# mengshanfeng/stencil-2

Measured on AMD Instinct MI355X. Metric: Jacobi3D Gcells/s (512^3/GPU weak scaling; halo-exchange GB/s in extra), higher is better.
Workload: dtype fp32

## Files before the change

csrc/include/stencil/kernels/stencil_ops.hpp:

```cpp
#pragma once
#include <cstdint>
#include <vector>

#include "stencil/core/geometry.hpp"
#include "stencil/domain/local_domain.hpp"

namespace stencil {

enum class StencilKind : int {
  Jacobi = 0,
  Astaroth = 1,
};

struct Spheres {
  bool enabled = false;
  Dim3 hot, cold;
  int64_t radius = 0;
  static Spheres jacobi(const Rect3 &cReg) {
    Spheres s;
    s.enabled = true;
    s.hot = Dim3(cReg.lo.x + (cReg.hi.x - cReg.lo.x) / 3, (cReg.lo.y + cReg.hi.y) / 2, (cReg.lo.z + cReg.hi.z) / 2);
    s.cold = Dim3(cReg.lo.x + (cReg.hi.x - cReg.lo.x) * 2 / 3, (cReg.lo.y + cReg.hi.y) / 2, (cReg.lo.z + cReg.hi.z) / 2);
    s.radius = (cReg.hi.x - cReg.lo.x) / 10;
    return s;
  }
};

struct StencilTune {
  int variant = 2;
  static constexpr int kMfma = 8;
  int ty = 2;
  int zchunk = 0;
  int nw = 8;
  int x3sched = 1;
  int x3parts = 0;
  float x3sphw = 0.45f;
  float x2sphw = 0.15f;
  bool x3sphchunk = true;
  int x3left = 3;
  bool x2early = true;
  int x2row = 1;
  int x2sched = 1;
  int x2xfast = 0;
  int x2reserve = 8;
  int reserveCUs = 0;
  bool x2lockstep = true;
  bool zslabRow = true;
  bool xcdRemap = true;
  bool nontemporal = true;
  bool alternateZ = true;
  int wrap = 0;
  uint64_t *publish = nullptr;
  uint64_t *blockClock = nullptr;
  int publishDepth = 0;
};
bool stencil7x2_row_kernel_used(const LocalDomain &dom, int64_t qi, const Rect3 &region, const StencilTune &tune);
int stencil7x2_wrappable_axes(const LocalDomain &dom, int64_t qi, int x2row = 1);

struct ForwardTarget {
  Dim3 dir;
  const LocalDomain *dst;
  Dim3 offset;
};

class HaloForwarder {
public:
  HaloForwarder(const LocalDomain &src, int64_t qi, const std::vector<ForwardTarget> &targets);
  ~HaloForwarder();
  HaloForwarder(const HaloForwarder &) = delete;
  HaloForwarder &operator=(const HaloForwarder &) = delete;
  const int *wm() const { return wm_; }
  const int *wp() const { return wp_; }
  int num_targets() const { return n_; }
  uint32_t mask(int parity) const { return mask_[parity]; }
  int64_t delta(int parity, int k) const { return delta_[parity][k]; }
  bool has_rest() const { return hasRest_; }
  void forward_rest(int parity, hipStream_t stream) const;
  static bool supported(const LocalDomain &dom, int64_t qi);

private:
  int wm_[3] = {0, 0, 0}, wp_[3] = {0, 0, 0};
  int n_ = 0;
  int dev_ = -1;
  uint32_t mask_[2] = {0, 0};
  int64_t delta_[2][27] = {};
  CopyPlan rest_[2];
  bool hasRest_ = false;
};
// ... 11 lines not shown
                    hipStream_t stream, const StencilTune &tune = StencilTune(), const HaloForwarder *fwd = nullptr);
bool stencil7x2_supported(const LocalDomain &dom, int64_t qi);
void stencil7x2_apply(const LocalDomain &dom, int64_t qi, const Rect3 &region, StencilKind kind, const Spheres &sph,
                      hipStream_t stream, const StencilTune &tune = StencilTune());
bool stencil7x3_supported(const LocalDomain &dom, int64_t qi, const Rect3 &region, const StencilTune &tune);
bool stencil7x3_apply(const LocalDomain &dom, int64_t qi, const Rect3 &region, StencilKind kind, const Spheres &sph,
                      hipStream_t stream, const StencilTune &tune);
void stencil7x2_apply_regions(const LocalDomain &dom, int64_t qi, const std::vector<Rect3> &regions, StencilKind kind,
                              const Spheres &sph, hipStream_t stream, int wrap = 0);
void stencil7x2_apply_exterior(const LocalDomain &dom, int64_t qi, const Rect3 &interior, StencilKind kind,
                               const Spheres &sph, hipStream_t stream, const StencilTune &tune = StencilTune());
struct X2Schedule {
  int parts = 0;
  int64_t blocks = 0;
  int rounds = 1;
};
inline X2Schedule x2_lockstep_schedule(int64_t slots, int64_t cols, int64_t nz, bool rounds = true) {
  X2Schedule r;
  if (slots < 4 || cols < 1) return r;
  if (cols > slots && rounds) {
    if (nz < 16) return r;
    r.rounds = int((cols + slots - 1) / slots);
    r.parts = 1;
    r.blocks = (cols + r.rounds - 1) / r.rounds;
    return r;
  }
  const int64_t P = (slots / 4 > cols || slots % cols == 0) ? slots / cols : 4;
  const int64_t cm = cols < slots / P ? cols : slots / P;
  if (cm < 1 || nz < 64 || nz / P < 16) return r;
  r.parts = int(P);
  r.blocks = P * cm;
  if (rounds && P == 4 && cm < cols && cols % 2 == 0) {
    const int64_t ch = cols / 2, P2 = slots / ch;
    if (P2 >= 2 && nz / P2 >= 16 && 16 * P2 * ch >= 15 * slots) {
      r.parts = int(P2);
      r.blocks = P2 * ch;
      r.rounds = 2;
    }
  }
  return r;
}

struct X3Schedule {
  int seg = 1, parts = 0;
  int64_t blocks = 0;
  int rounds = 1;
};
X3Schedule stencil7x3_schedule(bool xh, int64_t cols, int64_t nz, int64_t slots, const StencilTune &tune,
                               bool publishing);
struct X3LaunchInfo {
  bool supported = false;
  bool xh = false, ragged = false;
  int64_t cols = 0, slots = 0;
  int seg = 0, parts = 0;
  int64_t blocks = 0;
  int rounds = 0;
};
X3LaunchInfo stencil7x3_launch_info(const LocalDomain &dom, int64_t qi, const Rect3 &region, StencilKind kind,
                                    const Spheres &sph, const StencilTune &tune);

int stencil7_wrappable_axes(const LocalDomain &dom, int64_t qi);
bool stencil7_mfma_supported(const LocalDomain &dom, int64_t qi);
void stencil7_mfma_apply(const LocalDomain &dom, int64_t qi, const Rect3 &region, StencilKind kind, const Spheres &sph,
                         hipStream_t stream, const StencilTune &tune = StencilTune());
void stencil7_apply_regions(const LocalDomain &dom, int64_t qi, const std::vector<Rect3> &regions, StencilKind kind,
                            const Spheres &sph, hipStream_t stream, const StencilTune &tune = StencilTune());

void jacobi_init(const LocalDomain &dom, int64_t qi, const Rect3 &region, hipStream_t stream);
void astaroth_init(const LocalDomain &dom, int64_t qi, double period, hipStream_t stream);
void fill_value(const LocalDomain &dom, int64_t qi, double value, bool curr, hipStream_t stream);

}
```

csrc/python/bindings.cpp:

```cpp
#include <pybind11/functional.h>
#include <pybind11/pybind11.h>
#include <pybind11/stl.h>

#include <cstring>

#include "stencil/comm/proc_group.hpp"
#include "stencil/comm/ipc_event.hpp"
#include "stencil/comm/rccl_comm.hpp"
#include "stencil/domain/distributed_domain.hpp"
#include "stencil/kernels/copy.hpp"
#include "stencil/kernels/stencil_ops.hpp"
#include "stencil/models/stencil_model.hpp"
#include "stencil/rt/build_info.hpp"
#include "stencil/rt/statistics.hpp"
#include "stencil/topo/gpu_topology.hpp"
#include "stencil/topo/partition.hpp"
#include "stencil/topo/placement.hpp"
#include "stencil/topo/qap.hpp"

namespace py = pybind11;
using namespace stencil;

extern "C" {
struct DLDevice {
// ... 677 lines not shown
        py::arg("dd"), py::arg("domain"), py::arg("qi"));
  m.def("stencil7x2_apply",
        [](DistributedDomain &dd, size_t di, int64_t q, const Rect3 &region, StencilKind kind, bool spheres,
           uintptr_t stream, const StencilTune &tune) {
          STENCIL_REQUIRE(stencil7x2_supported(dd.domains().at(di), q),
                          "fused pairs need a device fp32/fp64 quantity, face radii >= 2 and the aligned layout");
          const Spheres s = spheres ? Spheres::jacobi(dd.get_compute_region()) : Spheres();
          stencil7x2_apply(dd.domains().at(di), q, region, kind, s, reinterpret_cast<hipStream_t>(stream), tune);
        },
        py::arg("dd"), py::arg("domain"), py::arg("qi"), py::arg("region"), py::arg("kind"), py::arg("spheres"),
        py::arg("stream"), py::arg("tune"), py::call_guard<py::gil_scoped_release>());
  py::class_<X3PlanInfo>(m, "X3PlanInfo")
      .def_readonly("parts", &X3PlanInfo::parts)
      .def_readonly("blocks", &X3PlanInfo::blocks)
      .def_readonly("groups", &X3PlanInfo::groups)
      .def_readonly("lockstep_groups", &X3PlanInfo::lockstepGroups)
      .def_readonly("rounds", &X3PlanInfo::rounds)
      .def_readonly("tabled", &X3PlanInfo::tabled)
      .def_readonly("steps", &X3PlanInfo::steps)
      .def_readonly("zb", &X3PlanInfo::zb)
      .def_readonly("l0", &X3PlanInfo::l0)
      .def_readonly("l1", &X3PlanInfo::l1)
      .def_readonly("odd", &X3PlanInfo::odd);
  m.def(
      "stencil7x3_plan",
      [](py::handle size, bool jacobi, py::object tune, int slots) {
        return stencil7x3_plan(to_dim3(size), jacobi, tune.is_none() ? StencilTune() : tune.cast<StencilTune>(), slots);
      },
      py::arg("size"), py::arg("jacobi"), py::arg("tune") = py::none(), py::arg("slots") = 256);
  m.def(
      "stencil7x3_schedule",
      [](bool xh, int64_t cols, int64_t nz, int64_t slots, py::object tune, bool publishing) {
        const X3Schedule r = stencil7x3_schedule(xh, cols, nz, slots,
                                                 tune.is_none() ? StencilTune() : tune.cast<StencilTune>(), publishing);
        return py::make_tuple(r.seg, r.parts, r.blocks, r.rounds);
      },
      py::arg("xh"), py::arg("cols"), py::arg("nz"), py::arg("slots"), py::arg("tune") = py::none(),
      py::arg("publishing") = false,
      "launch schedule of a fused-triple sweep (no GPU): (seg, parts, blocks, rounds) for the XH form (xh, columns with "
      "x halos) or the whole-row form over cols (row group, column) pairs of nz planes on `slots` resident blocks; seg "
      "1 = balanced split, 2 = lockstep parts plus second segments, 3 = lockstep rounds (XH form, not publishing)");
  m.def(
      "stencil7x3_launch_info",
      [](DistributedDomain &dd, size_t di, int64_t q, StencilKind kind, bool spheres, const StencilTune &tune) {
        const Spheres s = spheres ? Spheres::jacobi(dd.get_compute_region()) : Spheres();
        const LocalDomain &d = dd.domains().at(di);
        const X3LaunchInfo r = stencil7x3_launch_info(d, q, d.get_compute_region(), kind, s, tune);
        py::dict o;
        o["supported"] = r.supported;
        o["form"] = !r.supported ? "none" : (r.xh ? "xh" : "wrap");
        o["ragged"] = r.ragged;
        o["cols"] = r.cols;
        o["slots"] = r.slots;
        o["seg"] = r.seg;
        o["parts"] = r.parts;
        o["blocks"] = r.blocks;
        o["rounds"] = r.rounds;
        return o;
      },
      py::arg("dd"), py::arg("domain"), py::arg("qi"), py::arg("kind"), py::arg("spheres"), py::arg("tune"));
  m.def(
      "x2_lockstep_schedule",
      [](int64_t slots, int64_t cols, int64_t nz) {
        const X2Schedule r = x2_lockstep_schedule(slots, cols, nz);
        return py::make_tuple(r.parts, r.blocks, r.rounds);
      },
      py::arg("slots"), py::arg("cols"), py::arg("nz"),
      "lockstep schedule of the whole-row / two-chunk-column fused pairs: (z parts per row group, blocks, rounds of "
      "whole columns); (0, 0, 1) = balanced split");
  m.def("jacobi_spheres", [](const Rect3 &cReg) {
    Spheres s = Spheres::jacobi(cReg);
    return py::make_tuple(s.hot, s.cold, s.radius);
  });

  py::class_<StencilTune>(m, "StencilTune")
      .def(py::init<>())
      .def_readwrite("variant", &StencilTune::variant)
      .def_readwrite("ty", &StencilTune::ty)
      .def_readwrite("zchunk", &StencilTune::zchunk)
      .def_readwrite("xcd_remap", &StencilTune::xcdRemap)
      .def_readwrite("nontemporal", &StencilTune::nontemporal)
      .def_readwrite("alternate_z", &StencilTune::alternateZ)
      .def_readwrite("nw", &StencilTune::nw)
      .def_readwrite("x3sched", &StencilTune::x3sched)
      .def_readwrite("x2early", &StencilTune::x2early)
      .def_readwrite("x3parts", &StencilTune::x3parts)
      .def_readwrite("x3sphw", &StencilTune::x3sphw)
      .def_readwrite("x3sphchunk", &StencilTune::x3sphchunk)
      .def_readwrite("x3left", &StencilTune::x3left)
      .def_readwrite("x2sphw", &StencilTune::x2sphw)
      .def_property(
          "block_clock", [](const StencilTune &t) { return reinterpret_cast<uintptr_t>(t.blockClock); },
          [](StencilTune &t, uintptr_t p) { t.blockClock = reinterpret_cast<uint64_t *>(p); })
      .def_readwrite("x2row", &StencilTune::x2row)
      .def_readwrite("x2sched", &StencilTune::x2sched)
      .def_readwrite("x2reserve", &StencilTune::x2reserve)
      .def_readwrite("wrap", &StencilTune::wrap)
      .def_readwrite("x2lockstep", &StencilTune::x2lockstep)
      .def_readwrite("zslab_row", &StencilTune::zslabRow)
      .def_readwrite("x2xfast", &StencilTune::x2xfast);
  py::class_<StencilModelConfig>(m, "StencilModelConfig")
      .def(py::init<>())
      .def_readwrite("size", &StencilModelConfig::size)
      .def_readwrite("kind", &StencilModelConfig::kind)
      .def_readwrite("radius", &StencilModelConfig::radius)
      .def_readwrite("all_directions", &StencilModelConfig::allDirections)
      .def_readwrite("quantities", &StencilModelConfig::quantities)
      .def_readwrite("fp64", &StencilModelConfig::fp64)
      .def_readwrite("methods", &StencilModelConfig::methods)
      .def_readwrite("placement", &StencilModelConfig::placement)
      .def_readwrite("axis_cost", &StencilModelConfig::axisCost)
      .def_readwrite("partition", &StencilModelConfig::partition)
      .def_readwrite("gpus", &StencilModelConfig::gpus)
      .def_readwrite("overlap", &StencilModelConfig::overlap)
      .def_readwrite("auto_overlap", &StencilModelConfig::autoOverlap)
      .def_readwrite("use_graph", &StencilModelConfig::useGraph)
      .def_readwrite("forward", &StencilModelConfig::forward)
      .def_readwrite("temporal", &StencilModelConfig::temporal)
      .def_readwrite("wrap_self", &StencilModelConfig::wrapSelf)
      .def_readwrite("x_halo_align", &StencilModelConfig::xHaloAlign)
      .def_readwrite("shared_halo_line", &StencilModelConfig::sharedHaloLine)
      .def_readwrite("interior_align", &StencilModelConfig::interiorAlign)
      .def_readwrite("row_pad_lines", &StencilModelConfig::rowPadLines)
      .def_readwrite("wrap_axes_mask", &StencilModelConfig::wrapAxesMask)
      .def_readwrite("local_interior", &StencilModelConfig::localInterior)
      .def_readwrite("overlap_mode", &StencilModelConfig::overlapMode)
      .def_readwrite("transport", &StencilModelConfig::transport)
      .def_readwrite("self_test", &StencilModelConfig::selfTest)
      .def_property(
          "backend", [](const StencilModelConfig &c) { return c.backend; },
          [](StencilModelConfig &c, Backend b) {
            c.backend = b;
            c.setBackend = true;
          })
      .def_readwrite("tune", &StencilModelConfig::tune)
      .def_readwrite("astaroth_period", &StencilModelConfig::astarothPeriod);
  py::class_<StencilModel, std::shared_ptr<StencilModel>>(m, "StencilModel")
      .def(py::init([](const StencilModelConfig &c, std::shared_ptr<comm::ProcGroup> pg) {
             py::gil_scoped_release r;
// ... 36 lines not shown
```

csrc/src/kernels/stencil7x3.hip:

```cpp
#include <hip/hip_runtime.h>

#include <algorithm>
#include <map>
#include <mutex>
#include <utility>
#include <vector>
#include <cmath>
#include <cstring>

#include "stencil/kernels/stencil_ops.hpp"
#include "stencil/rt/hip_check.hpp"
#include "stencil_common.hpp"
#include "stencil_wave.hpp"

namespace stencil {

struct X3Seg {
  uint32_t s, e, s2, e2;
  bool odd;
  bool odd2;
};
template <typename T>
__device__ __forceinline__ X3Seg x3_segments(const StencilArgs<T> &a, const ZPartBounds &B, uint32_t lb, uint32_t nb,
                                             uint32_t ncols, uint32_t gy, uint32_t nzt) {
// ... 407 lines not shown
            for (int h = 0; h < H; ++h) {
              U1b[h] = U1c[h];
              U1c[h] = U1a[h];
              U2b[h] = U2c[h];
              U2c[h] = U2a[h];
            }
            if constexpr (EDGE) {
              U1Eb = U1Ec;
              U1Ec = U1Ea;
            }
            ++t;
            return true;
          };
          using I0 = std::integral_constant<int, 0>;
          using I1 = std::integral_constant<int, 1>;
          using I2 = std::integral_constant<int, 2>;
          using I3 = std::integral_constant<int, 3>;
          using L1 = std::integral_constant<int, (RM < 1 ? RM : 1)>;
          using L2 = std::integral_constant<int, (RM < 2 ? RM : 2)>;
          using LR = std::integral_constant<int, RM>;
          step(I0{}, L1{});
          step(I1{}, L1{});
          step(I2{}, L2{});
          step(I3{}, L2{});
          while (step(I0{}, LR{}) && step(I1{}, LR{}) && step(I2{}, LR{}) && step(I3{}, LR{})) {
          }
        };
        if (down)
          march(std::true_type{});
        else
          march(std::false_type{});
      }
    }
  };
  const unsigned long long clk0 = a.clk ? wall_clock64() : 0;
  const int role = (w >= 3 && w < NW - 3) ? 3 : ((w >= 2 && w < NW - 2) ? 2 : ((w >= 1 && w < NW - 1) ? 1 : 0));
  if (role == 3)
    body(std::integral_constant<int, 3>{});
  else if (role == 2)
    body(std::integral_constant<int, 2>{});
  else if (role == 1)
    body(std::integral_constant<int, 1>{});
  else
    body(std::integral_constant<int, 4>{});
  if (a.clk) {
    __syncthreads();
    if (lane == 0 && w == 0) {
      a.clk[2 * lb] = clk0;
      a.clk[2 * lb + 1] = wall_clock64();
    }
  }
}

template <int KIND, bool PUB>
__global__ __launch_bounds__(64 * 12, 3) __attribute__((amdgpu_waves_per_eu(3, 3))) void
stencil7x3_wrap_kernel(StencilArgs<float> a, ZPartBounds zbounds) {
  constexpr int NW = 12;
  using T = float;
  using NV = nf4;
  constexpr int V = 4, H = 2;
  constexpr int CS = 64 * V;
  constexpr int LS = V;
  constexpr int YO = NW - 6;
  constexpr int NC = 4;
  __shared__ NV cs[2][NW][H][64];
  __shared__ NV us[2][NW][H][64];
  __shared__ NV vs[2][NW][H][64];

  const uint32_t nb = gridDim.x;
  const uint32_t lb = a.remap ? xcd_remap(blockIdx.x, nb) : blockIdx.x;
  const int lane = threadIdx.x;
  const int w = __builtin_amdgcn_readfirstlane(int(threadIdx.y));
  const uint32_t nzt = uint32_t(a.hiz - a.loz);
  const X3Seg sg = x3_segments(a, zbounds, lb, nb, uint32_t(a.gy), uint32_t(a.gy), nzt);
  const bool lane0 = lane == 0, lane63 = lane == 63;
  const int wA = w > 0 ? w - 1 : 0, wB = w < NW - 1 ? w + 1 : NW - 1;
  const int xb = a.lox + lane * LS;
  const int zwn = a.wn[2], zwlo = a.wlo[2], zwhi = a.wlo[2] + a.wn[2];
  const __amdgpu_buffer_rsrc_t srcRsrc =
      __builtin_amdgcn_make_buffer_rsrc(const_cast<float *>(a.src), 0, -1, 0x00020000);
  auto zcl = [&](int zz) {
    zz += zz < zwlo ? zwn : 0;
    zz -= zz >= zwhi ? zwn : 0;
    return zz < 0 ? 0 : (zz > a.rawZm1 ? a.rawZm1 : zz);
  };
  auto body = [&](auto roleTag) {
    constexpr int R = decltype(roleTag)::value;
    bool odd = sg.odd;
    const bool pubOrder = PUB;
    for (int pp = 0; pp < 2; ++pp) {
      const int pass = pubOrder ? 1 - pp : pp;
      uint32_t s = pass == 0 ? sg.s : sg.s2;
      const uint32_t e = pass == 0 ? sg.e : sg.e2;
      if (pass == 1 && !pubOrder) odd = sg.odd2;
      while (s < e) {
        const uint32_t by = s / nzt;
        const int zo = int(s - by * nzt);
        const int nzs = int(min(nzt - uint32_t(zo), e - s));
        s += uint32_t(nzs);
        const int zs = a.loz + zo;
        const int ze = zs + nzs;
        bool down = pass == 0 && sg.odd;
        if (!pubOrder) {
          down = odd != (a.flip != 0);
          odd = !odd;
        }
        const int yblk = a.loy + YO * int(by);
        const int y = yblk - 3 + w;
        if (yblk >= a.hiy) continue;
        const bool outRow = R == 3 && y < a.hiy;
        int yw = y < a.wlo[1] ? y + a.wn[1] : (y >= a.wlo[1] + a.wn[1] ? y - a.wn[1] : y);
        yw = yw < 0 ? 0 : (yw > a.rawYm1 ? a.rawYm1 : yw);
        const uint32_t rowoff = uint32_t((yw * int64_t(a.px) + xb) * int64_t(sizeof(T)));
        const uint32_t outoff = uint32_t((y * int64_t(a.px) + xb) * int64_t(sizeof(T)));

        const int yh = a.r1sq - (y - a.hy) * (y - a.hy), yc = a.r1sq - (y - a.cy) * (y - a.cy);
        struct RowSph {
          int Dh, Dc;
          bool hit;
        };
        auto row_sph = [&](int P) -> RowSph {
          RowSph r{0, 0, false};
          if (KIND == 0) {
            r.Dh = yh - (P - a.hz) * (P - a.hz);
            r.Dc = yc - (P - a.cz) * (P - a.cz);
            r.hit = max(r.Dh, r.Dc) > 0;
          }
          return r;
        };
        auto sphere_row = [&](const RowSph &rs, NV(&o)[H]) {
          if (KIND == 0 && rs.hit) {
            const int Dh = rs.Dh, Dc = rs.Dc;
#pragma unroll
            for (int h = 0; h < H; ++h)
#pragma unroll
              for (int k = 0; k < V; ++k) {
                const int x = xb + h * CS + k;
                const bool hot = (x - a.hx) * (x - a.hx) < Dh;
                const bool cold = (x - a.cx) * (x - a.cx) < Dc;
                o[h][k] = hot ? T(1) : (cold ? T(0) : o[h][k]);
              }
          }
        };
        auto row_update = [&](const NV(&cm)[H], const NV(&up)[H], const NV(&dn)[H], const NV(&zp)[H], const NV(&zm)[H],
                              NV(&o)[H]) -> T {
          static_assert(H == 2, "two chunks per lane");
          const T r30 = rot_prev(cm[0][V - 1]), r31 = rot_prev(cm[1][V - 1]);
          const T l00 = rot_next(cm[0][0]), l01 = rot_next(cm[1][0]);
#pragma unroll
          for (int h = 0; h < H; ++h) {
            const T left = h == 0 ? (lane0 ? r31 : r30) : (lane0 ? r30 : r31);
            const T right = h == 0 ? (lane63 ? l01 : l00) : (lane63 ? l00 : l01);
            NV vpx, vmx;
#pragma unroll
            for (int k = 0; k < V; ++k) {
              vpx[k] = k < V - 1 ? cm[h][k + 1] : right;
              vmx[k] = k > 0 ? cm[h][k - 1] : left;
            }
            o[h] = div6v<T, NV, V>(sum6v<T, KIND>(vpx, vmx, dn[h], up[h], zp[h], zm[h]));
          }
          return T(1);
        };

        auto march = [&](auto downTag) {
          constexpr bool DOWN = decltype(downTag)::value;
          constexpr int dz = DOWN ? -1 : 1;
          const int z0 = DOWN ? ze - 1 : zs;
          NV C[NC][H];
          NV U1a[H], U1b[H], U1c[H];
          NV U2a[H], U2b[H], U2c[H];
          auto load_row = [&](int zz, int k) {
            const uint32_t po = uint32_t(zcl(zz)) * uint32_t(a.pxy) * uint32_t(sizeof(T));
#pragma unroll
            for (int h = 0; h < H; ++h)
              C[k][h] = __builtin_bit_cast(
                  NV, __builtin_amdgcn_raw_buffer_load_b128(srcRsrc, rowoff + uint32_t(h * CS * int(sizeof(T))), po, 0));
          };
          {
            const int zw = z0 - 3 * dz;
#pragma unroll
            for (int k = 0; k < NC - 1; ++k) load_row(zw + k * dz, k);
#pragma unroll
            for (int h = 0; h < H; ++h) {
              cs[0][w][h][lane] = C[1][h];
              U1a[h] = U1b[h] = U1c[h] = U2a[h] = U2b[h] = U2c[h] = C[1][h];
            }
            __syncthreads();
          }
          int buf = 0;
          int t = -4;
          auto step = [&](auto phase, auto lvTag) -> bool {
            constexpr int k = decltype(phase)::value;
            constexpr int LV = decltype(lvTag)::value;
            constexpr int s0 = k % NC, s1 = (k + 1) % NC, s2 = (k + 2) % NC, sn = (k + NC - 1) % NC;
            if (t >= nzs) return false;
            const int z = z0 + t * dz;
            load_row(z + NC * dz, sn);
            NV o[H];
            auto levels = [&]() {
              NV A1[H], B1[H], A2[H], B2[H], A3[H], B3[H];
              auto rd = [&](NV(&sh)[2][NW][H][64], NV(&A)[H], NV(&B)[H]) {
#pragma unroll
                for (int h = 0; h < H; ++h) {
                  A[h] = sh[buf][wA][h][lane];
                  B[h] = sh[buf][wB][h][lane];
                }
              };
              if constexpr (LV >= 1) {
                rd(cs, A1, B1);
                (void)row_update(C[s1], A1, B1, DOWN ? C[s0] : C[s2], DOWN ? C[s2] : C[s0], U1a);
                sphere_row(row_sph(z + 2 * dz), U1a);
#pragma unroll
                for (int h = 0; h < H; ++h) cs[buf ^ 1][w][h][lane] = C[s2][h];
#pragma unroll
                for (int h = 0; h < H; ++h) us[buf ^ 1][w][h][lane] = U1a[h];
              }
              if constexpr (LV >= 2) {
                rd(us, A2, B2);
                (void)row_update(U1c, A2, B2, DOWN ? U1b : U1a, DOWN ? U1a : U1b, U2a);
                sphere_row(row_sph(z + dz), U2a);
#pragma unroll
                for (int h = 0; h < H; ++h) vs[buf ^ 1][w][h][lane] = U2a[h];
              }
              if constexpr (LV >= 3) {
                rd(vs, A3, B3);
                (void)row_update(U2c, A3, B3, DOWN ? U2b : U2a, DOWN ? U2a : U2b, o);
                sphere_row(row_sph(z), o);
              }
            };
            levels();
            if constexpr (LV >= 3) {
              char *dp = outRow ? reinterpret_cast<char *>(a.dst + int64_t(z) * a.pxy) + outoff
                                : a.sink + lane * LS * int(sizeof(T));
#pragma unroll
              for (int h = 0; h < H; ++h) {
                NV *q = reinterpret_cast<NV *>(dp + h * CS * int(sizeof(T)));
                if (a.nt)
                  __builtin_nontemporal_store(o[h], q);
                else
                  *q = o[h];
              }
            }
            const int nbuf = buf ^ 1;
            if constexpr (LV < 1)
#pragma unroll
              for (int h = 0; h < H; ++h) cs[nbuf][w][h][lane] = C[s2][h];
            const bool pubStep = PUB && t >= 0 && (z < a.pubLo || z >= a.pubHi);
            if (pubStep) asm volatile("s_waitcnt vmcnt(0)" ::: "memory");
            __syncthreads();
            if (pubStep && lane == 0 && w == 0) {
              __builtin_amdgcn_fence(__ATOMIC_RELEASE, "");
              const unsigned long long cells =
                  (unsigned long long)(min(YO, a.hiy - yblk)) * (unsigned long long)(a.hix - a.lox);
              __hip_atomic_fetch_add(a.pub, cells, __ATOMIC_RELAXED, __HIP_MEMORY_SCOPE_SYSTEM);
            }
            buf = nbuf;
#pragma unroll
            for (int h = 0; h < H; ++h) {
              U1b[h] = U1c[h];
              U1c[h] = U1a[h];
              U2b[h] = U2c[h];
              U2c[h] = U2a[h];
            }
            ++t;
            return true;
          };
          using I0 = std::integral_constant<int, 0>;
          using I1 = std::integral_constant<int, 1>;
          using I2 = std::integral_constant<int, 2>;
          using I3 = std::integral_constant<int, 3>;
          using L1 = std::integral_constant<int, (R < 1 ? R : 1)>;
          using L2 = std::integral_constant<int, (R < 2 ? R : 2)>;
          using LR = std::integral_constant<int, R>;
          step(I0{}, L1{});
          step(I1{}, L1{});
          step(I2{}, L2{});
          step(I3{}, L2{});
          while (step(I0{}, LR{}) && step(I1{}, LR{}) && step(I2{}, LR{}) && step(I3{}, LR{})) {
          }
        };
        if (down)
          march(std::true_type{});
        else
          march(std::false_type{});
      }
    }
  };
  const unsigned long long clk0 = a.clk ? wall_clock64() : 0;
  const int role = (w >= 3 && w < NW - 3) ? 3 : ((w >= 2 && w < NW - 2) ? 2 : ((w >= 1 && w < NW - 1) ? 1 : 0));
  if (role == 3)
    body(std::integral_constant<int, 3>{});
  else if (role == 2)
    body(std::integral_constant<int, 2>{});
  else if (role == 1)
    body(std::integral_constant<int, 1>{});
  else
    body(std::integral_constant<int, 0>{});
  if (a.clk) {
    __syncthreads();
    if (lane == 0 && w == 0) {
      a.clk[2 * lb] = clk0;
      a.clk[2 * lb + 1] = wall_clock64();
    }
  }
}

template <typename T, int KIND> static const void *x3_wrap_kernel_ptr() {
  if constexpr (std::is_same<T, float>::value)
    return (const void *)stencil7x3_wrap_kernel<KIND, false>;
  else
    return nullptr;
}
template <typename T, int KIND> using X3XhKernel = void (*)(StencilArgs<T>, ZPartBounds);
template <typename T, int KIND, bool BIG, bool PUB> static X3XhKernel<T, KIND> x3_xh_kernel_ptr(bool rag) {
  return rag ? stencil7x3_xh_kernel<T, KIND, BIG, PUB, true> : stencil7x3_xh_kernel<T, KIND, BIG, PUB, false>;
}
template <typename T, int KIND> static X3XhKernel<T, KIND> x3_xh_kernel_ptr(bool big, bool pub, bool rag) {
  return big ? (pub ? x3_xh_kernel_ptr<T, KIND, true, true>(rag) : x3_xh_kernel_ptr<T, KIND, true, false>(rag))
             : (pub ? x3_xh_kernel_ptr<T, KIND, false, true>(rag) : x3_xh_kernel_ptr<T, KIND, false, false>(rag));
}

static int64_t x3_resident_blocks(const void *kernel, int threads) {
  static std::map<const void *, int64_t> cache;
  static std::mutex mu;
  std::lock_guard<std::mutex> lk(mu);
  auto it = cache.find(kernel);
  if (it != cache.end()) return it->second;
  int dev = 0, perCU = 0, cus = 256;
  (void)hipGetDevice(&dev);
  if (hipDeviceGetAttribute(&cus, hipDeviceAttributeMultiprocessorCount, dev) != hipSuccess) cus = 256;
  if (hipOccupancyMaxActiveBlocksPerMultiprocessor(&perCU, kernel, threads, 0) != hipSuccess || perCU <= 0) perCU = 1;
  (void)hipGetLastError();
  const int64_t r = int64_t(perCU) * cus;
  cache[kernel] = r;
  return r;
}

static std::map<int, char *> gX3Sinks;
static std::mutex gX3SinkMu;
static char *x3_sink(int dev, bool create) {
  std::lock_guard<std::mutex> lk(gX3SinkMu);
  char *&p = gX3Sinks[dev];
  if (!p && create) {
    int cur = 0;
    HIP_CHECK(hipGetDevice(&cur));
    HIP_CHECK(hipSetDevice(dev));
    HIP_CHECK(hipMalloc(reinterpret_cast<void **>(&p), 4096));
    HIP_CHECK(hipSetDevice(cur));
  }
  return p;
}

static int64_t x3_column_cells(int64_t elemSize) { return 2 * 64 * (16 / elemSize); }

bool stencil7x3_supported(const LocalDomain &dom, int64_t qi, const Rect3 &region, const StencilTune &tune) {
  if (dom.backend() != Backend::Device) return false;
  const int64_t es = dom.elem_size(qi);
  const bool f32 = dom.dtype(qi) == DType::F32 || (dom.dtype(qi) == DType::Bytes && es == 4);
  const bool f64 = dom.dtype(qi) == DType::F64 || (dom.dtype(qi) == DType::Bytes && es == 8);
  if (!f32 && !f64) return false;
  const Radius &rad = dom.radius();
  const Dim3 n = dom.size();
  const int wrapm = tune.wrap & 7;
  if (wrapm & 1) {
// ... 28 lines not shown
  X2Schedule ls = x2_lockstep_schedule(slots, cols, nz, rounds);
  if (tune.x3sched == 1) {
    ls = X2Schedule();
    double best = 1e30;
    for (int64_t P = 2; P <= 8; ++P) {
      if (tune.x3parts > 0 && P != tune.x3parts) continue;
      const int64_t cm = std::min<int64_t>(cols, slots / P);
      if (cm < 1 || nz / P < 16) continue;
      const int64_t blocksP = P * cm, left = cols - cm;
      const double cost = double(nz) / double(P) + 4 + (left > 0 ? double(left * nz) / double(blocksP) + 4 : 0);
      if (cost < best - 1e-9) {
        best = cost;
        ls.parts = int(P);
        ls.blocks = blocksP;
      }
    }
  }
  if (tune.x3sched == 1 && cols > slots && rounds) {
    ls = X2Schedule();
    double best = 1e30;
    for (int64_t R = (cols + slots - 1) / slots; R <= 4 * ((cols + slots - 1) / slots); ++R)
      for (int64_t P = 1; P <= 4; ++P) {
        const int64_t cm = (cols + R - 1) / R;
        if (P * cm > slots || nz / P < 16) continue;
        const double cost = double(R) * (double(nz) / double(P) + 4);
        if (cost < best - 1e-9) {
          best = cost;
          ls.parts = int(P);
          ls.blocks = P * cm;
          ls.rounds = int(R);
        }
      }
  }
  X3Schedule r;
  if (tune.x2lockstep && ls.parts > 0) {
    r.seg = ls.rounds > 1 ? 3 : 2;
    r.parts = ls.parts;
    r.blocks = ls.blocks;
    r.rounds = ls.rounds;
  } else {
    r.blocks = std::max<int64_t>(1, std::min<int64_t>(slots, cols * nz / 24));
  }
  return r;
}

struct X3Plan {
  int P;
  uint32_t blocks;
  ZPartBounds b;
  double steps;
};
template <typename T>
static X3Plan x3_plan(const StencilArgs<T> &a, bool jac, int64_t cols, int64_t slots, uint32_t blocks,
                      const StencilTune &tune) {
  constexpr int NW = 12, YO = NW - 6;
  constexpr double kUnsync = 1.2;
  const int64_t nz = a.hiz - a.loz;
  const float w = jac ? tune.x3sphw : 0.f;
  auto plan = [&](int P, int64_t nbP, ZPartBounds &b) -> double {
    b = ZPartBounds{};
    const int64_t cm = nbP / P;
    if (jac) sphere_part_bounds(b, a, std::min<int64_t>(cm, a.gy), P, NW, YO, 3, w);
    const int mode = tune.x3left;
    ZPartBounds bg = b, bl = b;
    const double tg = mode == 1 || mode == 3
                          ? balance_leftover(bg, a, nbP, cm, P, cols, a.gy, NW, YO, 3, w, 4, mode == 3 ? kUnsync : 1.0)
                          : -1;
    const double tl = mode == 2 || mode == 3 ? lockstep_leftover(bl, a, nbP, cm, P, cols, a.gy, NW, YO, 3, w, 4, 16) : -1;
    if (tl >= 0 && (tg < 0 || tl <= tg)) {
      b = bl;
      return tl;
    }
    if (tg >= 0) {
      b = bg;
      return tg;
    }
    const std::vector<double> mc = lockstep_part_costs(b, a, cm, P, a.gy, NW, YO, 3, w, 4);
    const double left = cols > cm ? double((cols - cm) * nz) * kUnsync / double(nbP) + 4 : 0;
    return *std::max_element(mc.begin(), mc.end()) + left;
  };
  X3Plan pl{a.zparts, blocks, ZPartBounds{}, 0};
  if (tune.x3sched == 1 && tune.x3parts <= 0 && tune.x3left != 0) {
    double best = -1;
    const bool sph = jac && a.r1sq > 0 && w > 0;
    for (int P = 2; P <= (sph ? kZPartMaxParts : 8); ++P) {
      const int64_t cm = std::min<int64_t>(cols, slots / P);
      if (cm < 1 || nz / P < 16) continue;
      ZPartBounds b;
      const double t = plan(P, P * cm, b);
      if (best < 0 || t < best - 1e-9) {
        best = t;
        pl = X3Plan{P, uint32_t(P * cm), b, t};
      }
    }
  } else {
    pl.steps = plan(a.zparts, int64_t(blocks), pl.b);
  }
  return pl;
}

template <typename T> struct X3Launch {
  StencilArgs<T> a;
  ZPartBounds zb;
  uint32_t blocks;
  bool big, rag;
  int64_t cols, slots;
};
template <typename T, int KIND, bool XH>
static X3Launch<T> x3_prepare(const LocalDomain &dom, int64_t qi, const Rect3 &region, const Spheres &sph,
                              const StencilTune &tune) {
  constexpr int NW = 12, YO = NW - 6;
  X3Launch<T> L{};
  StencilArgs<T> &a = L.a;
  a = make_args<T>(dom, qi, region, KIND == 0 ? StencilKind::Jacobi : StencilKind::Astaroth, sph);
  a.flip = tune.alternateZ ? (dom.parity() & 1) : 0;
  a.nt = tune.nontemporal ? 1 : 0;
  a.wrapm = tune.wrap & 7;
  if (!(a.wrapm & 2)) a.wn[1] = 0;
  if (!(a.wrapm & 4)) a.wn[2] = 0;
  a.x0 = a.lox;
  a.remap = tune.xcdRemap ? 1 : 0;
  a.sphchunk = tune.x3sphchunk ? 1 : 0;
  a.sphr = int(sph.radius);
  const int nx = a.hix - a.lox, ny = a.hiy - a.loy, nz = a.hiz - a.loz;
  const int cw = int(x3_column_cells(int64_t(sizeof(T))));
  a.gx = XH ? (nx + cw - 1) / cw : 1;
  a.xr = XH ? nx - (a.gx - 1) * cw : nx;
  const bool rag = XH && a.xr < cw;
  a.gy = (ny + YO - 1) / YO;
  const bool big = dom.buffer_bytes(qi) >= (int64_t(1) << 32) - 4096;
  const void *kern = XH ? (const void *)x3_xh_kernel_ptr<T, KIND>(big, false, rag) : x3_wrap_kernel_ptr<T, KIND>();
  const int64_t cols = int64_t(a.gx) * a.gy;
  const int64_t resident = x3_resident_blocks(kern, 64 * NW);
  int cus = 256;
  if (hipDeviceGetAttribute(&cus, hipDeviceAttributeMultiprocessorCount, dom.gpu()) != hipSuccess) cus = 256;
  const int64_t perCU = std::max<int64_t>(1, resident / std::max(1, cus));
  const int64_t slots = std::max<int64_t>(perCU, resident - perCU * std::min(tune.reserveCUs, cus / 2));
  if (tune.publish) {
    a.pub = reinterpret_cast<unsigned long long *>(tune.publish);
    a.pubLo = a.loz + tune.publishDepth;
    a.pubHi = a.hiz - tune.publishDepth;
    a.flip = 0;
  }
  const X3Schedule ls = stencil7x3_schedule(XH, cols, nz, slots, tune, tune.publish != nullptr);
  a.seg = ls.seg;
  uint32_t blocks = uint32_t(ls.blocks);
  if (ls.seg != 1) {
    a.zparts = ls.parts;
    a.zrounds = ls.rounds;
  }
  ZPartBounds &zb = L.zb;
  if (a.seg == 2) {
    static std::map<std::vector<int64_t>, X3Plan> cache;
    static std::mutex mu;
    int32_t wbits = 0;
    std::memcpy(&wbits, &tune.x3sphw, sizeof(wbits));
    const std::vector<int64_t> key{KIND, a.loy,  a.hiy, a.loz, a.hiz,          a.hy,        a.cy,
                                   a.hz, a.cz,   a.r1sq, int64_t(blocks), a.zparts, cols, a.gy,
                                   wbits, tune.x3left, tune.x3sched, tune.x3parts, slots};
    std::lock_guard<std::mutex> lk(mu);
    auto it = cache.find(key);
    if (it == cache.end()) it = cache.emplace(key, x3_plan(a, KIND == 0, cols, slots, blocks, tune)).first;
    a.zparts = it->second.P;
    blocks = it->second.blocks;
    zb = it->second.b;
  }
  a.sink = x3_sink(dom.gpu(), false);
  a.clk = reinterpret_cast<unsigned long long *>(tune.blockClock);
  L.blocks = blocks;
  L.big = big;
  L.rag = rag;
  L.cols = cols;
  L.slots = slots;
  return L;
}

template <typename T, int KIND, bool XH>
static void apply_x3_t(const LocalDomain &dom, int64_t qi, const Rect3 &region, const Spheres &sph, hipStream_t stream,
                       const StencilTune &tune) {
  constexpr int NW = 12;
  const X3Launch<T> L = x3_prepare<T, KIND, XH>(dom, qi, region, sph, tune);
  const StencilArgs<T> &a = L.a;
  const ZPartBounds &zb = L.zb;
  const uint32_t blocks = L.blocks;
  dom.set_device();
  STENCIL_REQUIRE(a.sink, "stencil7x3: no store sink on device " << dom.gpu() << " (stencil7x3_supported first)");
  if constexpr (XH || !std::is_same<T, float>::value) {
    const X3XhKernel<T, KIND> k = x3_xh_kernel_ptr<T, KIND>(L.big, a.pub != nullptr, L.rag);
    hipLaunchKernelGGL(k, dim3(blocks), dim3(64, NW), 0, stream, a, zb);
  } else {
    if (a.pub)
      hipLaunchKernelGGL((stencil7x3_wrap_kernel<KIND, true>), dim3(blocks), dim3(64, NW), 0, stream, a, zb);
    else
      hipLaunchKernelGGL((stencil7x3_wrap_kernel<KIND, false>), dim3(blocks), dim3(64, NW), 0, stream, a, zb);
  }
  HIP_CHECK(hipGetLastError());
}

X3PlanInfo stencil7x3_plan(const Dim3 &size, bool jacobi, const StencilTune &tune, int slots) {
  constexpr int YO = 6;
  StencilArgs<float> a{};
  a.hix = int(size.x);
  a.hiy = int(size.y);
  a.hiz = int(size.z);
  if (jacobi) {
    const Spheres s = Spheres::jacobi(Rect3(Dim3(0, 0, 0), size));
    a.hx = int(s.hot.x);
    a.hy = int(s.hot.y);
    a.hz = int(s.hot.z);
    a.cx = int(s.cold.x);
    a.cy = int(s.cold.y);
    a.cz = int(s.cold.z);
    a.r1sq = int((s.radius + 1) * (s.radius + 1));
  }
  a.gx = 1;
  a.gy = int((size.y + YO - 1) / YO);
  const int64_t cols = a.gy, nz = size.z;
  X3PlanInfo r;
  r.groups = int(cols);
  const X3Schedule ls = stencil7x3_schedule(false, cols, nz, slots, tune, tune.publish != nullptr);
  r.parts = ls.parts;
  r.blocks = ls.seg == 1 ? 0 : int(ls.blocks);
  r.rounds = ls.rounds;
  if (ls.seg != 2) return r;
  a.zparts = ls.parts;
  const X3Plan pl = x3_plan(a, jacobi, cols, slots, uint32_t(ls.blocks), tune);
  r.parts = pl.P;
  r.blocks = int(pl.blocks);
  r.lockstepGroups = int(pl.blocks) / pl.P;
  r.steps = pl.steps;
  r.tabled = pl.b.lon != 0;
  if (pl.b.on)
    for (int g = 0; g < std::min<int>(r.lockstepGroups, kZPartMaxCols); ++g)
      for (int q = 0; q + 1 < pl.P; ++q) r.zb.push_back(pl.b.zb[g][q]);
  if (r.tabled)
    for (uint32_t lb = 0; lb < pl.blocks; ++lb) {
      r.l0.push_back(pl.b.l0[lb]);
      r.l1.push_back(pl.b.l1[lb]);
      r.odd.push_back(int((pl.b.ldir[lb / 32] >> (lb % 32)) & 1));
    }
  return r;
}

bool stencil7x3_apply(const LocalDomain &dom, int64_t qi, const Rect3 &region, StencilKind kind, const Spheres &sph,
                      hipStream_t stream, const StencilTune &tune) {
  if (!stencil7x3_supported(dom, qi, region, tune)) return false;
  const bool jac = kind == StencilKind::Jacobi, xh = !(tune.wrap & 1);
  if (dom.elem_size(qi) == 8) {
    jac ? apply_x3_t<double, 0, true>(dom, qi, region, sph, stream, tune)
        : apply_x3_t<double, 1, true>(dom, qi, region, sph, stream, tune);
  } else if (xh) {
    jac ? apply_x3_t<float, 0, true>(dom, qi, region, sph, stream, tune)
        : apply_x3_t<float, 1, true>(dom, qi, region, sph, stream, tune);
  } else {
    jac ? apply_x3_t<float, 0, false>(dom, qi, region, sph, stream, tune)
        : apply_x3_t<float, 1, false>(dom, qi, region, sph, stream, tune);
  }
  return true;
}

template <typename T, int KIND, bool XH>
static X3LaunchInfo x3_launch_info_t(const LocalDomain &dom, int64_t qi, const Rect3 &region, const Spheres &sph,
                                     const StencilTune &tune) {
  const X3Launch<T> L = x3_prepare<T, KIND, XH>(dom, qi, region, sph, tune);
  X3LaunchInfo r;
  r.supported = true;
  r.xh = XH;
  r.ragged = L.rag;
  r.cols = L.cols;
  r.slots = L.slots;
  r.seg = L.a.seg;
  r.parts = L.a.seg == 1 ? 0 : L.a.zparts;
  r.blocks = int64_t(L.blocks);
  r.rounds = L.a.seg == 3 ? L.a.zrounds : 1;
  return r;
}

X3LaunchInfo stencil7x3_launch_info(const LocalDomain &dom, int64_t qi, const Rect3 &region, StencilKind kind,
                                    const Spheres &sph, const StencilTune &tune) {
  if (!stencil7x3_supported(dom, qi, region, tune)) return X3LaunchInfo();
  const bool jac = kind == StencilKind::Jacobi, xh = !(tune.wrap & 1);
  if (dom.elem_size(qi) == 8)
    return jac ? x3_launch_info_t<double, 0, true>(dom, qi, region, sph, tune)
               : x3_launch_info_t<double, 1, true>(dom, qi, region, sph, tune);
  if (xh)
    return jac ? x3_launch_info_t<float, 0, true>(dom, qi, region, sph, tune)
               : x3_launch_info_t<float, 1, true>(dom, qi, region, sph, tune);
  return jac ? x3_launch_info_t<float, 0, false>(dom, qi, region, sph, tune)
             : x3_launch_info_t<float, 1, false>(dom, qi, region, sph, tune);
}

}
```

Measured before the change: 1920.

## Add 14-wave 8-output-row variant of the x3 wrap kernel with auto selection

Templates the temporally-blocked x3 wrap kernel on wave count and adds a 14-wave form that produces 8 output rows per block instead of 6. This lowers the share of redundant halo rows recomputed across the three fused time levels, and it shrinks the intermediate shared buffers and masks sphere updates per chunk. Auto-selection picks 8 rows when ny divides by 8 and the z-partitioned column count fits the resident slots, but not when spheres are active, since kX3AutoRows8Spheres is false. Jacobi has spheres, so the default Jacobi path likely stays at 12 waves. The new form also trades occupancy (4 waves per EU) and adds planner complexity.

```diff
diff --git a/csrc/include/stencil/kernels/stencil_ops.hpp b/csrc/include/stencil/kernels/stencil_ops.hpp
--- a/csrc/include/stencil/kernels/stencil_ops.hpp
+++ b/csrc/include/stencil/kernels/stencil_ops.hpp
@@ -34,6 +34,7 @@
   int nw = 8;
   int x3sched = 1;
   int x3parts = 0;
+  int x3rows = 0;
   float x3sphw = 0.45f;
   float x2sphw = 0.15f;
   bool x3sphchunk = true;
@@ -151,6 +152,7 @@
   bool supported = false;
   bool xh = false, ragged = false;
   int64_t cols = 0, slots = 0;
+  int rows = 0;
   int seg = 0, parts = 0;
   int64_t blocks = 0;
   int rounds = 0;
diff --git a/csrc/python/bindings.cpp b/csrc/python/bindings.cpp
--- a/csrc/python/bindings.cpp
+++ b/csrc/python/bindings.cpp
@@ -753,6 +753,7 @@
         o["ragged"] = r.ragged;
         o["cols"] = r.cols;
         o["slots"] = r.slots;
+        o["rows"] = r.rows;
         o["seg"] = r.seg;
         o["parts"] = r.parts;
         o["blocks"] = r.blocks;
@@ -786,6 +787,7 @@
       .def_readwrite("x3sched", &StencilTune::x3sched)
       .def_readwrite("x2early", &StencilTune::x2early)
       .def_readwrite("x3parts", &StencilTune::x3parts)
+      .def_readwrite("x3rows", &StencilTune::x3rows)
       .def_readwrite("x3sphw", &StencilTune::x3sphw)
       .def_readwrite("x3sphchunk", &StencilTune::x3sphchunk)
       .def_readwrite("x3left", &StencilTune::x3left)
diff --git a/csrc/src/kernels/stencil7x3.hip b/csrc/src/kernels/stencil7x3.hip
--- a/csrc/src/kernels/stencil7x3.hip
+++ b/csrc/src/kernels/stencil7x3.hip
@@ -483,10 +483,11 @@
   }
 }
 
-template <int KIND, bool PUB>
-__global__ __launch_bounds__(64 * 12, 3) __attribute__((amdgpu_waves_per_eu(3, 3))) void
-stencil7x3_wrap_kernel(StencilArgs<float> a, ZPartBounds zbounds) {
-  constexpr int NW = 12;
+template <int KIND, bool PUB, int NW>
+__global__ __launch_bounds__(64 * NW, NW == 12 ? 3 : 4)
+    __attribute__((amdgpu_waves_per_eu(NW == 12 ? 3 : 4, NW == 12 ? 3 : 4))) void
+    stencil7x3_wrap_kernel(StencilArgs<float> a, ZPartBounds zbounds) {
+  static_assert(NW == 12 || NW == 14, "12 waves (6 output rows) or 14 (8 output rows)");
   using T = float;
   using NV = nf4;
   constexpr int V = 4, H = 2;
@@ -494,9 +495,10 @@
   constexpr int LS = V;
   constexpr int YO = NW - 6;
   constexpr int NC = 4;
+  constexpr int UO = NW == 12 ? 0 : 1, VO = NW == 12 ? 0 : 2;
   __shared__ NV cs[2][NW][H][64];
-  __shared__ NV us[2][NW][H][64];
-  __shared__ NV vs[2][NW][H][64];
+  __shared__ NV us[2][NW - 2 * UO][H][64];
+  __shared__ NV vs[2][NW - 2 * VO][H][64];
 
   const uint32_t nb = gridDim.x;
   const uint32_t lb = a.remap ? xcd_remap(blockIdx.x, nb) : blockIdx.x;
@@ -515,6 +517,16 @@
     zz -= zz >= zwhi ? zwn : 0;
     return zz < 0 ? 0 : (zz > a.rawZm1 ? a.rawZm1 : zz);
   };
+  int sphm = 0;
+  if constexpr (NW != 12 && KIND == 0) {
+#pragma unroll
+    for (int h = 0; h < H; ++h) {
+      const int lo = a.lox + h * CS, hi = lo + CS - 1;
+      sphm |= int(!a.sphchunk || (a.cx - a.sphr <= hi && a.cx + a.sphr >= lo)) << (2 * h);
+      sphm |= int(!a.sphchunk || (a.hx - a.sphr <= hi && a.hx + a.sphr >= lo)) << (2 * h + 1);
+    }
+    sphm = __builtin_amdgcn_readfirstlane(sphm);
+  }
   auto body = [&](auto roleTag) {
     constexpr int R = decltype(roleTag)::value;
     bool odd = sg.odd;
@@ -562,15 +574,35 @@
         auto sphere_row = [&](const RowSph &rs, NV(&o)[H]) {
           if (KIND == 0 && rs.hit) {
             const int Dh = rs.Dh, Dc = rs.Dc;
-#pragma unroll
-            for (int h = 0; h < H; ++h)
-#pragma unroll
-              for (int k = 0; k < V; ++k) {
-                const int x = xb + h * CS + k;
-                const bool hot = (x - a.hx) * (x - a.hx) < Dh;
-                const bool cold = (x - a.cx) * (x - a.cx) < Dc;
-                o[h][k] = hot ? T(1) : (cold ? T(0) : o[h][k]);
-              }
+            if constexpr (NW == 12) {
+#pragma unroll
+              for (int h = 0; h < H; ++h)
+#pragma unroll
+                for (int k = 0; k < V; ++k) {
+                  const int x = xb + h * CS + k;
+                  const bool hot = (x - a.hx) * (x - a.hx) < Dh;
+                  const bool cold = (x - a.cx) * (x - a.cx) < Dc;
+                  o[h][k] = hot ? T(1) : (cold ? T(0) : o[h][k]);
+                }
+            } else {
+              int xs = xb;
+              asm volatile("" : "+v"(xs));
+#pragma unroll
+              for (int h = 0; h < H; ++h) {
+                if ((sphm >> (2 * h)) & 1)
+#pragma unroll
+                  for (int k = 0; k < V; ++k) {
+                    const int x = xs + h * CS + k;
+                    o[h][k] = (x - a.cx) * (x - a.cx) < Dc ? T(0) : o[h][k];
+                  }
+                if ((sphm >> (2 * h + 1)) & 1)
+#pragma unroll
+                  for (int k = 0; k < V; ++k) {
+                    const int x = xs + h * CS + k;
+                    o[h][k] = (x - a.hx) * (x - a.hx) < Dh ? T(1) : o[h][k];
+                  }
+              }
+            }
           }
         };
         auto row_update = [&](const NV(&cm)[H], const NV(&up)[H], const NV(&dn)[H], const NV(&zp)[H], const NV(&zm)[H],
@@ -630,31 +662,35 @@
             NV o[H];
             auto levels = [&]() {
               NV A1[H], B1[H], A2[H], B2[H], A3[H], B3[H];
-              auto rd = [&](NV(&sh)[2][NW][H][64], NV(&A)[H], NV(&B)[H]) {
+              auto rd = [&](auto &sh, auto off, NV(&A)[H], NV(&B)[H]) {
+                constexpr int O = decltype(off)::value;
 #pragma unroll
                 for (int h = 0; h < H; ++h) {
-                  A[h] = sh[buf][wA][h][lane];
-                  B[h] = sh[buf][wB][h][lane];
+                  A[h] = sh[buf][wA - O][h][lane];
+                  B[h] = sh[buf][wB - O][h][lane];
                 }
               };
+              using O0 = std::integral_constant<int, 0>;
+              using OU = std::integral_constant<int, UO>;
+              using OV = std::integral_constant<int, VO>;
               if constexpr (LV >= 1) {
-                rd(cs, A1, B1);
+                rd(cs, O0{}, A1, B1);
                 (void)row_update(C[s1], A1, B1, DOWN ? C[s0] : C[s2], DOWN ? C[s2] : C[s0], U1a);
                 sphere_row(row_sph(z + 2 * dz), U1a);
 #pragma unroll
                 for (int h = 0; h < H; ++h) cs[buf ^ 1][w][h][lane] = C[s2][h];
 #pragma unroll
-                for (int h = 0; h < H; ++h) us[buf ^ 1][w][h][lane] = U1a[h];
+                for (int h = 0; h < H; ++h) us[buf ^ 1][w - UO][h][lane] = U1a[h];
               }
               if constexpr (LV >= 2) {
-                rd(us, A2, B2);
+                rd(us, OU{}, A2, B2);
                 (void)row_update(U1c, A2, B2, DOWN ? U1b : U1a, DOWN ? U1a : U1b, U2a);
                 sphere_row(row_sph(z + dz), U2a);
 #pragma unroll
-                for (int h = 0; h < H; ++h) vs[buf ^ 1][w][h][lane] = U2a[h];
+                for (int h = 0; h < H; ++h) vs[buf ^ 1][w - VO][h][lane] = U2a[h];
               }
               if constexpr (LV >= 3) {
-                rd(vs, A3, B3);
+                rd(vs, OV{}, A3, B3);
                 (void)row_update(U2c, A3, B3, DOWN ? U2b : U2a, DOWN ? U2a : U2b, o);
                 sphere_row(row_sph(z), o);
               }
@@ -736,11 +772,27 @@
   }
 }
 
-template <typename T, int KIND> static const void *x3_wrap_kernel_ptr() {
+template <typename T, int KIND> static const void *x3_wrap_kernel_ptr(int nw) {
   if constexpr (std::is_same<T, float>::value)
-    return (const void *)stencil7x3_wrap_kernel<KIND, false>;
+    return nw == 14 ? (const void *)stencil7x3_wrap_kernel<KIND, false, 14>
+                    : (const void *)stencil7x3_wrap_kernel<KIND, false, 12>;
   else
     return nullptr;
+}
+
+constexpr bool kX3AutoRows8 = true, kX3AutoRows8Spheres = false;
+static int x3_rows(bool wholeRows, bool publishing, bool spheres, int64_t ny, int64_t nz, int64_t slots,
+                   const StencilTune &tune) {
+  if (!wholeRows || publishing || tune.x3rows == 6) return 6;
+  if (tune.x3rows == 8) return 8;
+  if (!(spheres ? kX3AutoRows8Spheres : kX3AutoRows8) || ny % 8 != 0) return 6;
+  bool admissible = false;
+  for (int64_t P = 2; P <= 8; ++P) {
+    if ((tune.x3parts > 0 && P != tune.x3parts) || nz / P < 16) continue;
+    admissible = true;
+    if (P * (ny / 8) <= slots) return 8;
+  }
+  return admissible ? 6 : 8;
 }
 template <typename T, int KIND> using X3XhKernel = void (*)(StencilArgs<T>, ZPartBounds);
 template <typename T, int KIND, bool BIG, bool PUB> static X3XhKernel<T, KIND> x3_xh_kernel_ptr(bool rag) {
@@ -875,8 +927,8 @@
 };
 template <typename T>
 static X3Plan x3_plan(const StencilArgs<T> &a, bool jac, int64_t cols, int64_t slots, uint32_t blocks,
-                      const StencilTune &tune) {
-  constexpr int NW = 12, YO = NW - 6;
+                      const StencilTune &tune, int NW) {
+  const int YO = NW - 6;
   constexpr double kUnsync = 1.2;
   const int64_t nz = a.hiz - a.loz;
   const float w = jac ? tune.x3sphw : 0.f;
@@ -928,11 +980,12 @@
   uint32_t blocks;
   bool big, rag;
   int64_t cols, slots;
+  int nw;
 };
 template <typename T, int KIND, bool XH>
 static X3Launch<T> x3_prepare(const LocalDomain &dom, int64_t qi, const Rect3 &region, const Spheres &sph,
                               const StencilTune &tune) {
-  constexpr int NW = 12, YO = NW - 6;
+  STENCIL_REQUIRE(tune.x3rows == 0 || tune.x3rows == 6 || tune.x3rows == 8, "StencilTune::x3rows " << tune.x3rows);
   X3Launch<T> L{};
   StencilArgs<T> &a = L.a;
   a = make_args<T>(dom, qi, region, KIND == 0 ? StencilKind::Jacobi : StencilKind::Astaroth, sph);
@@ -950,15 +1003,24 @@
   a.gx = XH ? (nx + cw - 1) / cw : 1;
   a.xr = XH ? nx - (a.gx - 1) * cw : nx;
   const bool rag = XH && a.xr < cw;
-  a.gy = (ny + YO - 1) / YO;
   const bool big = dom.buffer_bytes(qi) >= (int64_t(1) << 32) - 4096;
-  const void *kern = XH ? (const void *)x3_xh_kernel_ptr<T, KIND>(big, false, rag) : x3_wrap_kernel_ptr<T, KIND>();
-  const int64_t cols = int64_t(a.gx) * a.gy;
-  const int64_t resident = x3_resident_blocks(kern, 64 * NW);
   int cus = 256;
   if (hipDeviceGetAttribute(&cus, hipDeviceAttributeMultiprocessorCount, dom.gpu()) != hipSuccess) cus = 256;
-  const int64_t perCU = std::max<int64_t>(1, resident / std::max(1, cus));
-  const int64_t slots = std::max<int64_t>(perCU, resident - perCU * std::min(tune.reserveCUs, cus / 2));
+  auto slots_of = [&](int nw) {
+    const void *kern =
+        XH ? (const void *)x3_xh_kernel_ptr<T, KIND>(big, false, rag) : x3_wrap_kernel_ptr<T, KIND>(nw);
+    const int64_t resident = x3_resident_blocks(kern, 64 * nw);
+    const int64_t perCU = std::max<int64_t>(1, resident / std::max(1, cus));
+    return std::max<int64_t>(perCU, resident - perCU * std::min(tune.reserveCUs, cus / 2));
+  };
+  constexpr bool wholeRows = !XH && std::is_same<T, float>::value;
+  const bool rows8 =
+      wholeRows && x3_rows(true, tune.publish != nullptr, KIND == 0 && a.r1sq > 0, ny, nz, slots_of(14), tune) == 8;
+  const int NW = rows8 ? 14 : 12, YO = NW - 6;
+  L.nw = NW;
+  a.gy = (ny + YO - 1) / YO;
+  const int64_t cols = int64_t(a.gx) * a.gy;
+  const int64_t slots = slots_of(NW);
   if (tune.publish) {
     a.pub = reinterpret_cast<unsigned long long *>(tune.publish);
     a.pubLo = a.loz + tune.publishDepth;
@@ -980,10 +1042,10 @@
     std::memcpy(&wbits, &tune.x3sphw, sizeof(wbits));
     const std::vector<int64_t> key{KIND, a.loy,  a.hiy, a.loz, a.hiz,          a.hy,        a.cy,
                                    a.hz, a.cz,   a.r1sq, int64_t(blocks), a.zparts, cols, a.gy,
-                                   wbits, tune.x3left, tune.x3sched, tune.x3parts, slots};
+                                   wbits, tune.x3left, tune.x3sched, tune.x3parts, slots, NW};
     std::lock_guard<std::mutex> lk(mu);
     auto it = cache.find(key);
-    if (it == cache.end()) it = cache.emplace(key, x3_plan(a, KIND == 0, cols, slots, blocks, tune)).first;
+    if (it == cache.end()) it = cache.emplace(key, x3_plan(a, KIND == 0, cols, slots, blocks, tune, NW)).first;
     a.zparts = it->second.P;
     blocks = it->second.blocks;
     zb = it->second.b;
@@ -1001,7 +1063,6 @@
 template <typename T, int KIND, bool XH>
 static void apply_x3_t(const LocalDomain &dom, int64_t qi, const Rect3 &region, const Spheres &sph, hipStream_t stream,
                        const StencilTune &tune) {
-  constexpr int NW = 12;
   const X3Launch<T> L = x3_prepare<T, KIND, XH>(dom, qi, region, sph, tune);
   const StencilArgs<T> &a = L.a;
   const ZPartBounds &zb = L.zb;
@@ -1010,18 +1071,22 @@
   STENCIL_REQUIRE(a.sink, "stencil7x3: no store sink on device " << dom.gpu() << " (stencil7x3_supported first)");
   if constexpr (XH || !std::is_same<T, float>::value) {
     const X3XhKernel<T, KIND> k = x3_xh_kernel_ptr<T, KIND>(L.big, a.pub != nullptr, L.rag);
-    hipLaunchKernelGGL(k, dim3(blocks), dim3(64, NW), 0, stream, a, zb);
+    STENCIL_REQUIRE(L.nw == 12, "stencil7x3: the XH form has 12 waves");
+    hipLaunchKernelGGL(k, dim3(blocks), dim3(64, 12), 0, stream, a, zb);
   } else {
+    STENCIL_REQUIRE(L.nw == 12 || (L.nw == 14 && !a.pub), "stencil7x3: " << L.nw << " waves");
     if (a.pub)
-      hipLaunchKernelGGL((stencil7x3_wrap_kernel<KIND, true>), dim3(blocks), dim3(64, NW), 0, stream, a, zb);
+      hipLaunchKernelGGL((stencil7x3_wrap_kernel<KIND, true, 12>), dim3(blocks), dim3(64, 12), 0, stream, a, zb);
+    else if (L.nw == 14)
+      hipLaunchKernelGGL((stencil7x3_wrap_kernel<KIND, false, 14>), dim3(blocks), dim3(64, 14), 0, stream, a, zb);
     else
-      hipLaunchKernelGGL((stencil7x3_wrap_kernel<KIND, false>), dim3(blocks), dim3(64, NW), 0, stream, a, zb);
+      hipLaunchKernelGGL((stencil7x3_wrap_kernel<KIND, false, 12>), dim3(blocks), dim3(64, 12), 0, stream, a, zb);
   }
   HIP_CHECK(hipGetLastError());
 }
 
 X3PlanInfo stencil7x3_plan(const Dim3 &size, bool jacobi, const StencilTune &tune, int slots) {
-  constexpr int YO = 6;
+  const int YO = tune.x3rows == 8 && tune.publish == nullptr ? 8 : 6, NW = YO + 6;
   StencilArgs<float> a{};
   a.hix = int(size.x);
   a.hiy = int(size.y);
@@ -1047,7 +1112,7 @@
   r.rounds = ls.rounds;
   if (ls.seg != 2) return r;
   a.zparts = ls.parts;
-  const X3Plan pl = x3_plan(a, jacobi, cols, slots, uint32_t(ls.blocks), tune);
+  const X3Plan pl = x3_plan(a, jacobi, cols, slots, uint32_t(ls.blocks), tune, NW);
   r.parts = pl.P;
   r.blocks = int(pl.blocks);
   r.lockstepGroups = int(pl.blocks) / pl.P;
@@ -1092,6 +1157,7 @@
   r.ragged = L.rag;
   r.cols = L.cols;
   r.slots = L.slots;
+  r.rows = L.nw - 6;
   r.seg = L.a.seg;
   r.parts = L.a.seg == 1 ? 0 : L.a.zparts;
   r.blocks = int64_t(L.blocks);
diff --git a/profiles/r7/clk.py b/profiles/r7/clk.py
--- /dev/null
+++ b/profiles/r7/clk.py
@@ -0,0 +1,27 @@
+import sys
+import torch
+import stencil2_amd as st
+
+clk = torch.zeros(1024, dtype=torch.int64, device="cuda")
+t = st.StencilTune()
+t.block_clock = clk.data_ptr()
+for kv in sys.argv[1:]:
+    k, v = kv.split("=")
+    setattr(t, k, type(getattr(t, k))(float(v)))
+m = st.Jacobi3D((512, 512, 512), gpus=[0], temporal=3, tune=t, use_graph=False)
+m.init()
+res = []
+for i in range(8):
+    clk.zero_()
+    m.run(3)
+    m.synchronize()
+    c = clk.view(-1, 2).cpu()
+    used = (c[:, 1] > 0).nonzero().flatten()
+    nb = int(used.max()) + 1
+    t0 = int(c[used, 0].min())
+    d = sorted((int(c[b, 1]) - int(c[b, 0])) / 100.0 for b in range(nb))
+    sweep = (int(c[used, 1].max()) - t0) / 100.0
+    skew = (int(c[used, 0].max()) - t0) / 100.0
+    res.append((nb, sweep, d[0], d[nb // 2], d[-1], skew))
+for r in res[3:]:
+    print("blocks %d sweep %.1f us; block min %.1f median %.1f max %.1f; start skew %.1f" % r, flush=True)
```

After: 1868. 0.973x the previous value.
